# rbarile17/kelpie

Measured on AMD Instinct MI355X. Metric: candidate explanations evaluated/sec (incl. post-train) + rank-delta match rate, higher is better.
Workload: dtype bf16x3 (fp32-emulated)

## Files before the change

### include/kelpie_hip.h

```cpp
#ifndef KELPIE_HIP_H
#define KELPIE_HIP_H

#include <stddef.h>
#include <stdint.h>

#ifdef __cplusplus
extern "C" {
#endif

#define KP_OK 0
#define KP_EINVAL (-22)
#define KP_ENOMEM (-12)
#define KP_EDEVICE (-5)
#define KP_ENOTSUP (-95)
#define KP_INLINE 1

#define KP_MODEL_TRANSE 0
#define KP_MODEL_COMPLEX 1
#define KP_MODEL_CONVE 2

#define KP_OPT_ADAGRAD 0
#define KP_OPT_ADAM 1
#define KP_OPT_SGD 2

// ... 104 lines not shown
                        int32_t D, int32_t d, float xavier_std, int32_t n, const int32_t* R_base,
                        const int32_t* R_pt, const uint8_t* want, int32_t epochs, int32_t ratio,
                        int64_t n_entities, float* x_base, float* x_pt, int32_t* out);

int kp_rng_transe_calls_async(const uint8_t* torch_state, size_t torch_len, uint32_t* np_key, int32_t* np_pos,
                              int32_t normal_cap, int32_t D, int32_t d, float xavier_std, int32_t n,
                              const int32_t* R_base, const int32_t* R_pt, const uint8_t* want, int32_t epochs,
                              int32_t ratio, int64_t n_entities, float* x_base, float* x_pt, int32_t* out);

int kp_rng_torch_take(uint8_t* torch_state, size_t torch_len, int32_t* taken);

int kp_rng_wait(void);

int kp_rng_conve_masks(uint8_t* torch_state, size_t torch_len, int32_t n_steps, const int32_t* rows_per_step,
                       int32_t n_seg, const int32_t* seg_elems, const double* seg_keep, uint32_t* out_words);

int kp_rng_conve_masks_enqueue(uint8_t* torch_state, size_t torch_len, int32_t n_steps, const int32_t* rows_per_step,
                               int32_t n_seg, const int32_t* seg_elems, const double* seg_keep,
                               uint32_t* out_words);

int kp_last_timing(const kp_ctx* ctx, double* device_seconds, double* hot_kernel_seconds,
                   int64_t* hot_kernel_launches, double* hot_work_units);

int kp_hot_intervals(const kp_ctx* ctx, int64_t cap, double* out, int64_t* n);

typedef struct kp_graph kp_graph;
int kp_graph_create(int32_t n_ent, int64_t n_triples, const int32_t* triples, kp_graph** out);
void kp_graph_destroy(kp_graph* g);
const char* kp_graph_last_error(void);

int kp_graph_bfs(const kp_graph* g, int32_t n_src, const int32_t* src, int32_t* dist);

int kp_graph_set_classes(kp_graph* g, const int64_t* cls_off, const int32_t* cls);

int kp_graph_dijkstra_pairs(const kp_graph* g, int32_t n, const int32_t* src, const int32_t* dst, double* out);

typedef struct kp_view kp_view;
typedef struct kp_sched_batch kp_sched_batch;
int kp_view_create(int32_t kelpie, int32_t n_rel, int32_t original, const int32_t* base, int32_t n,
                   const int32_t* extra, int32_t m, kp_view** out);
void kp_view_destroy(kp_view* v);
int kp_sched_batch_create(kp_sched_batch** out);
void kp_sched_batch_destroy(kp_sched_batch* b);

int kp_sched_add_calls(kp_sched_batch* b, int32_t n, kp_view* const* views, const int32_t* rel, const uint8_t* flags,
                       const int32_t* cand_off, const int32_t* cands, int32_t* slot_idx, int32_t* n_rows,
// ... 14 lines not shown
```

### kelpie_amd/_lib.py

```python
from __future__ import annotations

import ctypes as C
import os
import sys
import weakref

import numpy as np

_HERE = os.path.dirname(os.path.abspath(__file__))
LIB_PATH = os.environ.get("KELPIE_HIP_LIB", os.path.join(_HERE, "libkelpie_hip.so"))

KP_MODEL = {"TransE": 0, "ComplEx": 1, "ConvE": 2}
KP_INLINE = 1
KP_OPT = {"Adagrad": 0, "Adam": 1, "SGD": 2}

EXPORTS = ["kp_ctx_create", "kp_ctx_destroy", "kp_last_error", "kp_posttrain_rank", "kp_all_scores",
           "kp_convertible", "kp_mt19937_discard", "kp_last_timing", "kp_version", "kp_rng_bernoulli_bits",
           "kp_rng_transe_epochs", "kp_rng_transe_enqueue", "kp_rng_wait", "kp_rng_batch_close", "kp_rng_batch_wait", "kp_rng_conve_masks", "kp_rng_conve_masks_enqueue", "kp_graph_create", "kp_graph_destroy",
           "kp_graph_last_error", "kp_graph_bfs", "kp_graph_set_classes", "kp_graph_dijkstra_pairs",
           "kp_predict_tails", "kp_dp_relevance", "kp_criage_relevance", "kp_hot_intervals", "kp_rng_normal",
           "kp_rng_transe_calls", "kp_train_epoch", "kp_read_tables", "kp_view_create", "kp_view_destroy",
           "kp_sched_batch_create", "kp_sched_batch_destroy", "kp_sched_add_calls", "kp_sched_pack",
           "kp_gather_i32", "kp_rng_transe_calls_async", "kp_rng_torch_take", "kp_conve_train_begin",
           "kp_conve_train_step", "kp_conve_train_read", "kp_host_alloc", "kp_host_free"]


class ModelDesc(C.Structure):
    _fields_ = [("model", C.c_int32), ("n_ent", C.c_int32), ("n_rel2", C.c_int32), ("dim", C.c_int32),
                ("entity", C.c_void_p), ("relation", C.c_void_p), ("conv_w", C.c_void_p), ("conv_b", C.c_void_p),
                ("fc_w", C.c_void_p), ("fc_b", C.c_void_p), ("bn_alpha", C.c_void_p), ("bn_beta", C.c_void_p),
                ("norm_p", C.c_int32)]


class HP(C.Structure):
    _fields_ = [("optimizer", C.c_int32), ("epochs", C.c_int32), ("batch_size", C.c_int32), ("lr", C.c_float),
                ("beta1", C.c_float), ("beta2", C.c_float), ("eps", C.c_float), ("reg_weight", C.c_float),
                ("margin", C.c_float), ("neg_ratio", C.c_int32), ("label_smoothing", C.c_float),
                ("hidden_dropout", C.c_float), ("input_dropout", C.c_float), ("fmap_dropout", C.c_float),
                ("reg_kind", C.c_int32)]


KP_REG = {"N3": 0, "N2": 1}


class Batch(C.Structure):
    _fields_ = [("n_slots", C.c_int32), ("x0", C.c_void_p), ("row_off", C.c_void_p), ("rows", C.c_void_p),
                ("rng_off", C.c_void_p), ("rng", C.c_void_p), ("pred", C.c_void_p), ("filt_off", C.c_void_p),
# ... 35 lines not shown
        L.kp_graph_destroy.restype = None
        L.kp_graph_last_error.restype = C.c_char_p
        L.kp_graph_bfs.argtypes = [C.c_void_p, C.c_int32, C.c_void_p, C.c_void_p]
        L.kp_graph_set_classes.argtypes = [C.c_void_p, C.c_void_p, C.c_void_p]
        L.kp_graph_dijkstra_pairs.argtypes = [C.c_void_p, C.c_int32, C.c_void_p, C.c_void_p, C.c_void_p]
        L.kp_rng_bernoulli_bits.argtypes = [C.c_void_p, C.c_size_t, C.c_uint64, C.c_double, C.c_void_p]
        L.kp_rng_transe_epochs.argtypes = [C.c_void_p, C.c_size_t, C.c_void_p, C.c_void_p, C.c_int32, C.c_int32,
                                           C.c_int32, C.c_int64, C.c_void_p]
        L.kp_rng_transe_enqueue.argtypes = L.kp_rng_transe_epochs.argtypes
        L.kp_rng_wait.argtypes = []
        L.kp_rng_batch_close.argtypes = [C.POINTER(C.c_int64)]
        L.kp_rng_batch_wait.argtypes = [C.c_int64]
        L.kp_train_epoch.argtypes = [C.c_void_p, C.POINTER(HP), C.c_int32, C.c_void_p, C.c_void_p, C.c_int32]
        L.kp_read_tables.argtypes = [C.c_void_p, C.c_void_p, C.c_void_p]
        L.kp_rng_normal.argtypes = [C.c_void_p, C.c_size_t, C.c_int64, C.c_float, C.c_float, C.c_int32, C.c_void_p]
        L.kp_rng_transe_calls.argtypes = [C.c_void_p, C.c_size_t, C.c_void_p, C.c_void_p, C.c_int32, C.c_int32,
                                          C.c_int32, C.c_float, C.c_int32, C.c_void_p, C.c_void_p, C.c_void_p,
                                          C.c_int32, C.c_int32, C.c_int64, C.c_void_p, C.c_void_p, C.c_void_p]
        L.kp_rng_conve_masks.argtypes = [C.c_void_p, C.c_size_t, C.c_int32, C.c_void_p, C.c_int32, C.c_void_p,
                                         C.c_void_p, C.c_void_p]
        L.kp_rng_conve_masks_enqueue.argtypes = L.kp_rng_conve_masks.argtypes
        L.kp_last_timing.argtypes = [C.c_void_p, C.POINTER(C.c_double), C.POINTER(C.c_double),
                                     C.POINTER(C.c_int64), C.POINTER(C.c_double)]
        L.kp_hot_intervals.argtypes = [C.c_void_p, C.c_int64, C.c_void_p, C.POINTER(C.c_int64)]
        L.kp_version.restype = C.c_char_p
        L.kp_view_create.argtypes = [C.c_int32, C.c_int32, C.c_int32, C.c_void_p, C.c_int32, C.c_void_p, C.c_int32,
                                     C.POINTER(C.c_void_p)]
        L.kp_view_destroy.argtypes = [C.c_void_p]
        L.kp_view_destroy.restype = None
        L.kp_sched_batch_create.argtypes = [C.POINTER(C.c_void_p)]
        L.kp_sched_batch_destroy.argtypes = [C.c_void_p]
        L.kp_sched_batch_destroy.restype = None
        L.kp_sched_add_calls.argtypes = [C.c_void_p, C.c_int32, C.c_void_p, C.c_void_p, C.c_void_p, C.c_void_p,
                                         C.c_void_p, C.c_void_p, C.c_void_p, C.c_void_p, C.c_void_p]
        L.kp_sched_pack.argtypes = [C.c_void_p, C.c_int32, C.c_void_p, C.c_void_p, C.c_int64, C.c_void_p,
                                    C.c_int64]
        L.kp_gather_i32.argtypes = [C.c_int32, C.c_void_p, C.c_void_p, C.c_void_p, C.c_int64]
        L.kp_rng_transe_calls_async.argtypes = L.kp_rng_transe_calls.argtypes
        L.kp_rng_torch_take.argtypes = [C.c_void_p, C.c_size_t, C.c_void_p]
        L.kp_conve_train_begin.argtypes = [C.c_void_p] * 5
        L.kp_conve_train_step.argtypes = [C.c_void_p, C.c_int32] + [C.c_void_p] * 6 + [C.c_float, C.c_float,
                                                                                      C.c_int32]
        L.kp_conve_train_read.argtypes = [C.c_void_p] * 9
        _LIB = L
    return _LIB

# ... 273 lines not shown
        check(lib().kp_dp_relevance(self.h, len(it), _ptr(it), float(epsilon), float(lambd), int(step_sign),
                                    int(rel_sign), _ptr(out)), self.h)
        return out

    def criage_relevance(self, items, ent_ids, tails_off, tails):
        it = np.ascontiguousarray(np.asarray(items, dtype=np.int32).reshape(-1, 5))
        ents = np.ascontiguousarray(ent_ids, dtype=np.int32)
        off = np.ascontiguousarray(tails_off, dtype=np.int32)
        tl = np.ascontiguousarray(np.asarray(tails, dtype=np.int32).reshape(-1, 2)) if len(tails) \
            else np.zeros((1, 2), np.int32)
        out = np.zeros(len(it), np.float64)
        status = np.zeros(len(it), np.int32)
        check(lib().kp_criage_relevance(self.h, len(it), _ptr(it), len(ents), _ptr(ents), _ptr(off), _ptr(tl),
                                        _ptr(out), _ptr(status)), self.h)
        return out, status

    def hot_intervals(self) -> np.ndarray:
        n = C.c_int64()
        check(lib().kp_hot_intervals(self.h, 0, None, C.byref(n)), self.h)
        out = np.zeros((max(1, n.value), 2), np.float64)
        check(lib().kp_hot_intervals(self.h, n.value, _ptr(out), C.byref(n)), self.h)
        return out[:n.value]

    def last_timing(self):
        a, b, n, w = C.c_double(), C.c_double(), C.c_int64(), C.c_double()
        check(lib().kp_last_timing(self.h, C.byref(a), C.byref(b), C.byref(n), C.byref(w)), self.h)
        return {"device_s": a.value, "hot_s": b.value, "hot_launches": n.value, "hot_work": w.value}


class Graph:

    def __init__(self, n_ent: int, triples):
        t = np.ascontiguousarray(np.asarray(triples, dtype=np.int32).reshape(-1, 3))
        h = C.c_void_p()
        self._lib = lib()
        self._check(self._lib.kp_graph_create(int(n_ent), len(t), _ptr(t), C.byref(h)))
        self._h = h
        self.n_ent = int(n_ent)

    def _check(self, rc):
        if rc != 0:
            raise KelpieHipError(f"libkelpie_hip error {rc}: {self._lib.kp_graph_last_error().decode()}")

    def __del__(self):
        h = getattr(self, "_h", None)
        if h is not None and h.value:
# ... 143 lines not shown
```

### kelpie_amd/csrc/kp_api.hip

```cpp
#include <cmath>
#include <cstdio>
#include <cstdlib>

#include "kp_common.hpp"

int cx_pick_db(int dim);

static thread_local std::string g_tls_err;

template <class F>
static int guarded(kp_ctx* c, F&& f) {
  try {
    f();
    if (c) c->err.clear();
    return KP_OK;
  } catch (const KpError& e) {
    if (c) c->err = e.msg;
    g_tls_err = e.msg;
    return e.code;
  } catch (const std::bad_alloc&) {
    if (c) c->err = "host out of memory";
    g_tls_err = "host out of memory";
    return KP_ENOMEM;
  } catch (...) {
// ... 77 lines not shown
    c->te_norm = m->norm_p == 1 ? 1 : 2;
    KP_HIP(hipSetDevice(device));
    KP_HIP(hipDeviceGetAttribute(&c->n_cu, hipDeviceAttributeMultiprocessorCount, device));
    (void)kp_time_base(device, nullptr);
    if (m->model == KP_MODEL_COMPLEX || m->model == KP_MODEL_CONVE) {
      KP_REQUIRE(m->model != KP_MODEL_COMPLEX || m->dim % 2 == 0, "ComplEx: row width must be even ([Re | Im])");
      int db = cx_pick_db(m->dim);
      KP_REQUIRE(db > 0, "row width > 400 not supported yet for ComplEx / ConvE");
      c->dp = 16 * db;
    } else {
      c->dp = round_up(m->dim, 16);
    }
    c->attn_mode = 1;
    if (const char* a = std::getenv("KP_ATTN")) c->attn_mode = std::strcmp(a, "f32") == 0 ? 0 : 1;
    c->cv_fused = 1;
    if (const char* a = std::getenv("KP_CV_FUSED")) c->cv_fused = std::atoi(a) != 0;
    c->cv_shared = 1;
    if (const char* a = std::getenv("KP_CV_SHARED")) c->cv_shared = std::atoi(a) != 0;
    if (const char* a = std::getenv("KP_CV_RANK")) c->cv_rank64 = std::strcmp(a, "f32") != 0;
    if (const char* a = std::getenv("KP_CV_DX")) c->cv_dx_block = std::strcmp(a, "block") == 0;
    if (const char* a = std::getenv("KP_TE_RANK")) c->te_rank64 = std::strcmp(a, "f32") != 0;
    if (const char* a = std::getenv("KP_ATTN_PART"))
      c->attn_part = std::strcmp(a, "streamk") == 0 ? 1 : std::strcmp(a, "ranges") == 0 ? 2 : 0;
    KP_HIP(hipStreamCreateWithFlags(&c->stream, hipStreamNonBlocking));
    {
      hipMemPool_t pool = device_pool(device);
      for (DevBuf* d : c->buffers()) {
        d->s = c->stream;
        d->pool = pool;
      }
    }
    KP_HIP(hipEventCreate(&c->ev0));
    KP_HIP(hipEventCreate(&c->ev1));
    upload_padded(c, &c->dE, m->entity, m->n_ent, m->dim, c->dp);
    upload_padded(c, &c->dR, m->relation, m->n_rel2, m->dim, c->dp);
    if (m->model == KP_MODEL_CONVE) {
      KP_REQUIRE(m->conv_w && m->conv_b && m->fc_w && m->fc_b && m->bn_alpha && m->bn_beta,
                 "ConvE: missing frozen layers");
      KP_REQUIRE(m->dim % 20 == 0 && m->dim / 20 >= 3, "ConvE: dim must be 20*h with h >= 3");
      c->hidden = 32 * 38 * (m->dim / 20 - 2);
      upload_plain(&c->d_conv_w, m->conv_w, 32 * 9);
      upload_plain(&c->d_conv_b, m->conv_b, 32);
      upload_plain(&c->d_fc_w, m->fc_w, (size_t)m->dim * c->hidden);
      upload_plain(&c->d_fc_b, m->fc_b, m->dim);
      upload_plain(&c->d_bn_a, m->bn_alpha, 1 + 32 + m->dim);
      upload_plain(&c->d_bn_b, m->bn_beta, 1 + 32 + m->dim);
// ... 211 lines not shown
                        const int32_t* tails_off, const int32_t* tails, double* out, int32_t* status) {
  if (!c || n < 0 || n_ents < 0 || (n > 0 && (!items || !out || !status || n_ents == 0)) ||
      (n_ents > 0 && (!ent_ids || !tails_off)))
    return KP_EINVAL;
  return guarded(c, [&] {
    if (n == 0) return;
    KP_HIP(hipSetDevice(c->device));
    criage_relevance(c, n, items, n_ents, ent_ids, tails_off, tails, out, status);
  });
}


int kp_hot_intervals(const kp_ctx* c, int64_t cap, double* out, int64_t* n) {
  if (!c || cap < 0 || (cap > 0 && !out)) return KP_EINVAL;
  const int64_t have = (int64_t)(c->hot_iv.size() / 2);
  if (n) *n = have;
  for (int64_t i = 0; i < std::min(cap, have); ++i) {
    out[2 * i] = c->hot_iv[2 * i];
    out[2 * i + 1] = c->hot_iv[2 * i + 1];
  }
  return KP_OK;
}

int kp_last_timing(const kp_ctx* c, double* dev_s, double* hot_s, int64_t* hot_n, double* hot_w) {
  if (!c) return KP_EINVAL;
  if (hot_w) *hot_w = c->timing.hot_work;
  if (dev_s) *dev_s = c->timing.device_s;
  if (hot_s) *hot_s = c->timing.hot_s;
  if (hot_n) *hot_n = c->timing.hot_launches;
  return KP_OK;
}

}
```

### kelpie_amd/csrc/kp_attn.hpp

```cpp
#pragma once
#if (defined(KP_ATTN_NODMA) || defined(KP_DIAG_M0SAVE)) && !defined(KP_DIAGNOSTIC_BUILD)
#error "KP_ATTN_NODMA is a timing-only diagnostic (wrong results): build it with make diag"
#endif
#include <algorithm>

#include "kp_common.hpp"

namespace kpattn {

#ifdef KP_ATTN_STAMPS
__device__ unsigned long long g_attn_stamps[8];
#define KP_STAMP(v) v = __builtin_amdgcn_s_memtime()
#else
#define KP_STAMP(v) (void)0
#endif

constexpr float kNegInf = -__builtin_huge_valf();

__device__ __forceinline__ float cx_q(const float* __restrict__ lhs, const float* __restrict__ rel, int d,
                                      int half) {
  if (d < half) {
    float ac = __fmul_rn(lhs[d], rel[d]);
    float be = __fmul_rn(lhs[d + half], rel[d + half]);
    return __fsub_rn(ac, be);
  } else if (d < 2 * half) {
    int i = d - half;
    float ae = __fmul_rn(lhs[i], rel[d]);
    float bc = __fmul_rn(lhs[d], rel[i]);
// ... 21 lines not shown
  return v;
}
__device__ __forceinline__ float lds_rd32(uint32_t addr) {
  float v;
  asm volatile("ds_read_b32 %0, %1" : "=v"(v) : "v"(addr));
  return v;
}
template <int N>
__device__ __forceinline__ void lgkm_wait() {
  asm volatile("s_waitcnt lgkmcnt(%0)" ::"n"(N));
}
__device__ __forceinline__ f32x4 tied(f32x4 v) {
  asm volatile("" : "+v"(v));
  return v;
}
__device__ __forceinline__ float tied(float v) {
  asm volatile("" : "+v"(v));
  return v;
}

enum { ATT_SOFTMAX_O = 0, ATT_SOFTMAX = 1, ATT_BCE_O = 2 };
constexpr float kMargin = 40.0f;

struct AttnWork {
  int ktq;
  int per_wg;
  int n_parts;
  int ranges;
};

template <int DB, int MODE>
__global__ __launch_bounds__(256, 1) void kp_attn(const float* __restrict__ E, int n_ent,
                                                  const float* __restrict__ Qpre, int nq, AttnWork wk,
                                                  float* __restrict__ out_m, float* __restrict__ out_l,
                                                  float* __restrict__ out_O, const float* __restrict__ qscale,
                                                  float ylo) {
  constexpr bool WITH_O = MODE != ATT_SOFTMAX;
  constexpr int DP = 16 * DB;
  constexpr int NSUB = 2;
  constexpr int KT = 16 * NSUB;
  constexpr int F4_ROW = DP / 4;
  constexpr int SEGS = (F4_ROW + 63) / 64;
  constexpr int S = 256 * SEGS + 4;
  extern __shared__ __attribute__((aligned(16))) float lds[];

  const int tid = threadIdx.x;
  const int lane = tid & 63;
  const int w = __builtin_amdgcn_readfirstlane(tid >> 6);
  const int g = lane >> 4, c = lane & 15;
  int key_begin = 0, key_end = 0;
  const uint32_t lds0 = (uint32_t)(uintptr_t)(__attribute__((address_space(3))) float*)lds;

// ... 207 lines not shown
              make_float4(O[4 * m][r], O[4 * m + 1][r], O[4 * m + 2][r], O[4 * m + 3][r]);
#pragma unroll
        for (int k = 0; k < DB % 4; ++k) dst[64 * (DB / 4) + 16 * k + i] = O[4 * (DB / 4) + k][r];
      }
    }
  }
  if (kt1 == wk.ktq && valid) {
    for (int pp = part + 1; pp < wk.n_parts; ++pp) {
      const size_t o = (size_t)pp * nq + q;
      if (g == 0 && MODE != ATT_BCE_O) {
        out_m[o] = kNegInf;
        out_l[o] = 0.f;
      }
      if (WITH_O) {
        float* dst = out_O + o * DP;
        for (int d = 4 * g; d < DP; d += 16) *reinterpret_cast<float4*>(dst + d) = make_float4(0.f, 0.f, 0.f, 0.f);
      }
    }
  }
  it += kt1 - kt0;
  }
}

struct AttnPlan {
  AttnWork wk;
  int n_wg;
};
inline AttnPlan attn_plan(int nq, int n_ent, int slots) {
  const int QT = (nq + 63) / 64, ktq = (n_ent + 31) / 32;
  const long long total = (long long)QT * ktq;
  long long per = (total + slots - 1) / slots;
  per = std::max<long long>(per, (ktq + 14) / 15);
  per = std::max<long long>(per, 1);
  AttnPlan p{};
  p.n_wg = (int)((total + per - 1) / per);
  p.wk.ktq = ktq;
  p.wk.per_wg = (int)per;
  int parts = 1;
  for (int qt = 0; qt < QT; ++qt) {
    const long long w0 = ((long long)qt * ktq) / per, w1 = ((long long)(qt + 1) * ktq - 1) / per;
    parts = std::max(parts, (int)(w1 - w0 + 1));
  }
  p.wk.n_parts = parts;
  return p;
}

inline AttnPlan attn_plan_ranges(int nq, int n_ent, int slots) {
  const int QT = (nq + 63) / 64, ktq = (n_ent + 31) / 32;
  const int n_wg = std::max(8, slots / 8 * 8);
  int best_s = 1;
  long long best = -1;
  for (int S = 1; S <= std::min(16, ktq); ++S) {
    const long long rounds = ((long long)QT * S + n_wg - 1) / n_wg;
    const long long cost = rounds * ((ktq + S - 1) / S + 2);
    if (best < 0 || cost < best) {
      best = cost;
      best_s = S;
    }
  }
  AttnPlan p{};
  p.wk.ktq = ktq;
  p.wk.per_wg = 0;
  p.wk.n_parts = best_s;
  p.wk.ranges = best_s;
  p.n_wg = (int)std::min<long long>(n_wg, ((long long)QT * best_s + 7) / 8 * 8);
  return p;
}

constexpr size_t attn_lds_bytes(int DB) {
  return 2u * 32u * (256u * ((4u * DB + 63u) / 64u) + 4u) * sizeof(float);
}

}
```

### kelpie_amd/csrc/kp_attn3.hpp

```cpp
#pragma once
#include <type_traits>

#include "kp_attn.hpp"

#ifdef KP_ATTN3_STAMPS
#ifndef KP_DIAGNOSTIC_BUILD
#error "KP_ATTN3_STAMPS is a diagnostic build (make diag / tools/attn_micro.sh)"
#endif
__device__ unsigned long long g_attn3_stamps[8];
#define KP3_STAMP(v) v = __builtin_amdgcn_s_memtime()
#define KP3_ACC(i, a, b) st_acc[i] += (b) - (a)
#else
#define KP3_STAMP(v) (void)0
#define KP3_ACC(i, a, b) (void)0
#endif

#ifdef KP_ATTN3_CLOCK
#ifndef KP_DIAGNOSTIC_BUILD
#error "KP_ATTN3_CLOCK is a diagnostic build (tools/attn_micro.sh)"
#endif
__device__ unsigned long long g_attn3_clock[4096][4];
#endif

#ifndef KP_O_AHEAD
// ... 885 lines not shown
    double* pre = reinterpret_cast<double*>(c->e3pre.ensure(sizeof(double) * (size_t)(ntiles + 1) * DP));
    hipLaunchKernelGGL((kp_tile_sums<DP>), dim3((unsigned)ntiles), dim3((DP + 63) / 64 * 64), 0, c->stream, c->dE,
                       c->n_ent, ts);
    KP_HIP(hipGetLastError());
    hipLaunchKernelGGL((kp_tile_prefix<DP>), dim3((DP + 63) / 64), dim3(64), 0, c->stream, ts, ntiles, pre);
    KP_HIP(hipGetLastError());
    c->e3pre_ready = true;
  }
  return c->e3pre.as<double>();
}

template <int DB, int MODE = ATT_SOFTMAX_O>
int attn3_wpc(kp_ctx* c) {
  static_assert(MODE == ATT_SOFTMAX_O || MODE == ATT_BCE_O, "attn3_wpc: the launched O mode");
  int& slot = c->attn3_wpc[MODE == ATT_BCE_O ? 1 : 0];
  if (slot <= 0) {
    int n = 0;
    KP_HIP(hipOccupancyMaxActiveBlocksPerMultiprocessor(&n, kp_attn3<DB, MODE>, 256, attn3_lds_bytes(DB)));
    slot = std::max(1, n);
  }
  return slot;
}

inline AttnPlan attn_plan_ctx(const kp_ctx* c, int nq, int n_ent, int slots) {
  const AttnPlan sk = attn_plan(nq, n_ent, slots);
  if (c->attn_mode != 1 || c->attn_part == 1) return sk;
  const AttnPlan r = attn_plan_ranges(nq, n_ent, slots);
  if (c->attn_part == 2) return r;
  const long long QT = (nq + 63) / 64, S = r.wk.ranges, ktq = r.wk.ktq;
  const long long n_wg = std::max(8, slots / 8 * 8);
  const long long cost_r = (QT * S + n_wg - 1) / n_wg * ((ktq + S - 1) / S + 2);
  const long long cost_sk = (long long)sk.wk.per_wg + 2;
  (void)n_ent;
  return 100 * cost_r <= 140 * cost_sk ? r : sk;
}

template <int DB, int MODE>
void launch_attn3(kp_ctx* c, int n_ent, const float* Q, int nq, const AttnPlan& plan, float* m, float* l, float* O,
                  const float* qscale, float ylo) {
  KP_REQUIRE(n_ent == c->n_ent, "attn3: key count differs from the table's (tile prefix sums)");
  KP_REQUIRE((long long)(n_ent + 31) / 32 * 32 * split3_row_bytes(16 * DB) + 1024 < (1LL << 31),
             "attn3: table too large for the 32-bit buffer descriptor of the split image");
  const uint8_t* E3 = split3_image<DB>(c);
  const double* pre = tile_prefix<DB>(c);
  hipLaunchKernelGGL((kp_attn3<DB, MODE>), dim3(plan.n_wg), dim3(256), attn3_lds_bytes(DB), c->stream, E3, n_ent, Q,
                     nq, plan.wk, m, l, O, qscale, ylo, pre);
  KP_HIP(hipGetLastError());
}

}
```

### kelpie_amd/csrc/kp_common.hpp

```cpp
#pragma once

#include <hip/hip_runtime.h>

#include <algorithm>
#include <array>
#include <cstdint>
#include <cstring>
#include <mutex>
#include <string>
#include <tuple>
#include <utility>
#include <vector>

#include "../../include/kelpie_hip.h"

typedef float f32x4 __attribute__((ext_vector_type(4)));

#define KP_WAVE 64

struct KpError {
  int code;
  std::string msg;
};

// ... 148 lines not shown
  hipEvent_t ev0 = nullptr, ev1 = nullptr;
  int model = 0;
  int n_ent = 0, n_rel2 = 0, dim = 0, dp = 0;
  int hidden = 0;
  float* dE = nullptr;
  float* dR = nullptr;
  float* d_conv_w = nullptr;
  float* d_conv_b = nullptr;
  float* d_fc_w = nullptr;
  float* d_fc_wt = nullptr;
  float* d_fc_b = nullptr;
  float* d_bn_a = nullptr;
  float* d_bn_b = nullptr;
  std::vector<float> hE;
  RankWs rank;
  ComplexWs cx;
  TranseWs te;
  ConveWs cv;
  std::string err;
  Timing timing;
  bool time_hot = true;
  int attn_mode = 0;
  int attn_part = 0;
  bool e3_ready = false;
  bool e3pre_ready = false;
  bool eT_ready = false;
  int cv_fused = 1;
  int cv_rank64 = 1;
  int cv_dx_block = 0;
  int te_norm = 2;
  int te_rank64 = 1;
  bool cvf_ready = false;
  int cv_shared = 1;
  bool cv_shared_ready = false;
  int attn3_wpc[2] = {0, 0};
  kp_train_state* train = nullptr;
  kp_cv_train* cvtrain = nullptr;
  std::vector<hipEvent_t> evpool;
  std::vector<std::pair<double, double>> hot_pairs;
  std::vector<double> hot_iv;
  std::vector<DevBuf*> buffers() {
    std::vector<DevBuf*> v;
    auto add = [&v](auto list) { v.insert(v.end(), list.begin(), list.end()); };
    add(ImageBufs::all());
    add(rank.all());
    add(cx.all());
// ... 109 lines not shown
```

### kelpie_amd/csrc/kp_complex.hip

```cpp
#include <algorithm>
#include <cstdio>
#include <cstdlib>
#include <cmath>
#include <unordered_map>

#include "kp_attn.hpp"
#include "kp_attn3.hpp"
#include "kp_posttrain.hpp"

namespace {
using namespace kpattn;

struct CxPlan {
  int b, q_begin, q_count, t_begin, t_count, cnt_l, cnt_r, pad;
};
struct CxQuery {
  int rel, c, ck, tg_begin, tg_count, pad0, pad1, pad2;
};
struct CxTail {
  int pair, c;
};


__global__ void kp_cx_qpair(const float* __restrict__ E, const float* __restrict__ R, int dp, int half,
// ... 577 lines not shown
  int32_t* dTg = upload(c, c->cx.targets, targets.data(), targets.size());
  int2* dPairs = upload(c, c->cx.pairs, pairs.data(), pairs.size());
  int4* dActs = upload(c, c->cx.acts, acts.data(), acts.size());
  int4* dStepQ = upload(c, c->cx.stepq, stepq.data(), std::max<size_t>(1, stepq.size()));
  int4* dStepT = upload(c, c->cx.stept, stept.data(), std::max<size_t>(1, stept.size()));
  float* dContrib = reinterpret_cast<float*>(c->cx.contrib.ensure(sizeof(float) * (size_t)std::max(1, max_items) * DP));
  const int npq = (int)pqs.size(), npairs = (int)pairs.size();
  float* dTsum = reinterpret_cast<float*>(c->cx.tsum.ensure(sizeof(float) * (size_t)std::max(npq, 1) * DP));
  float* dQpair = reinterpret_cast<float*>(c->cx.qpair.ensure(sizeof(float) * (size_t)std::max(npairs, 1) * DP));
  float* dLsef = reinterpret_cast<float*>(c->cx.lsef.ensure(sizeof(float) * (size_t)std::max(npairs, 1)));

  const Rank64Dev r64 = rank64_buffers(c, ns);
  int32_t* dPred = upload(c, c->rank.pred, bt->pred, (size_t)ns * 3);
  const RankDev rk = upload_rank_inputs(c, bt);

  const int half = c->dim / 2;
  KP_HIP(hipEventRecord(c->ev0, c->stream));
  if (npq > 0) {
    hipLaunchKernelGGL(kp_cx_tsum, dim3(npq), dim3(128), 0, c->stream, c->dE, DP, dPq, npq, dTg, dTsum);
    KP_HIP(hipGetLastError());
  }
  int slots_attn = 0;
  CX_DISPATCH(DBV, slots_attn = attn_slots_db<DB>(c));
  const AttnPlan plan_pairs = attn_plan_ctx(c, std::max(npairs, 1), c->n_ent, slots_attn);
  const int split_pairs = plan_pairs.wk.n_parts;
  size_t att_rows = (size_t)std::max(npairs, 1) * split_pairs;
  std::vector<AttnPlan> step_plan(T);
  for (int t = 0; t < T; ++t) {
    const int nq = q_off[t + 1] - q_off[t];
    step_plan[t] = attn_plan_ctx(c, std::max(nq, 1), c->n_ent, slots_attn);
    att_rows = std::max(att_rows, (size_t)nq * step_plan[t].wk.n_parts);
  }
  float* dAm = reinterpret_cast<float*>(c->cx.am.ensure(sizeof(float) * att_rows));
  float* dAl = reinterpret_cast<float*>(c->cx.al.ensure(sizeof(float) * att_rows));
  float* dAO = reinterpret_cast<float*>(c->cx.ao.ensure(sizeof(float) * att_rows * DP));
  float* dQs = reinterpret_cast<float*>(c->cx.qs.ensure(sizeof(float) * (size_t)std::max(max_nq, 1) * DP));
  if (npairs > 0) {
    hipLaunchKernelGGL(kp_cx_qpair, dim3(npairs), dim3(128), 0, c->stream, c->dE, c->dR, DP, half, dPairs, npairs,
                       dQpair);
    KP_HIP(hipGetLastError());
    CX_DISPATCH(DBV, launch_attn<DB>(c, false, dQpair, npairs, plan_pairs, dAm, dAl, nullptr));
    hipLaunchKernelGGL(kp_cx_lse_merge, dim3((npairs + 255) / 256), dim3(256), 0, c->stream, npairs, split_pairs, dAm,
                       dAl, dLsef);
    KP_HIP(hipGetLastError());
  }

  CxOpt opt{};
  opt.kind = hp->optimizer;
  opt.lr = hp->lr;
  opt.b1 = hp->beta1;
  opt.b2 = hp->beta2;
  opt.eps = hp->eps;
  opt.one_minus_b1 = (float)(1.0 - (double)hp->beta1);
// ... 99 lines not shown
```

### kelpie_amd/csrc/kp_conve.hip

```cpp
#include <cstdio>
#include <cmath>
#include <unordered_map>

#include "kp_attn.hpp"
#include "kp_attn3.hpp"
#include "kp_cv_fused.hpp"
#include "kp_posttrain.hpp"

int cx_pick_db(int dim);

namespace {
using namespace kpattn;

using kpcvf::CvBits;
struct CvInst {
  int slot, rel, b, pos;
  CvBits mb;
  int tail_begin, tail_count;
};
struct CvFInst {
  int slot, fp, b, pos;
  CvBits mb;
};
struct CvAct {
// ... 863 lines not shown
  int4* dFch = upload(c, c->cv.fchunks, fchunks.data(), std::max<size_t>(1, fchunks.size()));
  float* dFpart = reinterpret_cast<float*>(c->cv.fpart.ensure(sizeof(float) * (size_t)std::max(1, max_fch) * c->dim));
  CvBits* dEncBits = upload(c, c->cv.enc_bits, enc_bits.data(), std::max<size_t>(1, enc_bits.size()));
  float* dgs = reinterpret_cast<float*>(c->cv.gscale.ensure(sizeof(float) * (size_t)std::max<size_t>(1, kinst.size())));
  {
    std::vector<float> gsv(kinst.size());
    for (size_t i = 0; i < kinst.size(); ++i) gsv[i] = 1.0f / (float)((long long)kinst[i].b * (long long)(K + 1));
    if (!gsv.empty())
      KP_HIP(hipMemcpyAsync(dgs, gsv.data(), sizeof(float) * gsv.size(), hipMemcpyHostToDevice, c->stream));
  }
  int attn_slots = c->n_cu * (DBV <= 13 ? 2 : 1);
  if (c->attn_mode == 1) {
    switch (DBV) {
      case 4: attn_slots = c->n_cu * attn3_wpc<4, ATT_BCE_O>(c); break;
      case 8: attn_slots = c->n_cu * attn3_wpc<8, ATT_BCE_O>(c); break;
      case 13: attn_slots = c->n_cu * attn3_wpc<13, ATT_BCE_O>(c); break;
      case 16: attn_slots = c->n_cu * attn3_wpc<16, ATT_BCE_O>(c); break;
      case 25: attn_slots = c->n_cu * attn3_wpc<25, ATT_BCE_O>(c); break;
      default: throw KpError{KP_ENOTSUP, "ConvE: unsupported padded dimension"};
    }
  }
  std::vector<AttnPlan> step_plan(T);
  size_t o_rows = 1;
  for (int t = 0; t < T; ++t) {
    const int nk = kin_off[t + 1] - kin_off[t];
    step_plan[t] = attn_plan_ctx(c, std::max(nk, 1), K, attn_slots);
    o_rows = std::max(o_rows, (size_t)nk * step_plan[t].wk.n_parts);
  }
  float* dO = reinterpret_cast<float*>(c->cv.o.ensure(sizeof(float) * o_rows * DP));
  float* ddfc = reinterpret_cast<float*>(c->cv.dfc.ensure(sizeof(float) * (size_t)mk * c->dim));
  float* dgk = reinterpret_cast<float*>(c->cv.gk.ensure(sizeof(float) * (size_t)mk));
  float* ddflat = reinterpret_cast<float*>(c->cv.dflat.ensure(sizeof(float) * (size_t)(fused ? 1 : mk) * c->hidden));
  float* ddl = reinterpret_cast<float*>(c->cv.dl.ensure(sizeof(float) * (size_t)n_dl * mk * DP));
  float* dWt = conve_fc_wt(c);
  const float s_in = kc.has_in ? kc.scale_in : 1.0f, s_fm = kc.has_fm ? kc.scale_fm : 1.0f;

  CvOpt opt{};
  opt.lr = hp->lr;
  opt.b1 = hp->beta1;
  opt.b2 = hp->beta2;
  opt.eps = hp->eps;
  opt.one_minus_b1 = (float)(1.0 - (double)hp->beta1);
  opt.one_minus_b2 = (float)(1.0 - (double)hp->beta2);
  int64_t launches = 0;
  c->hot_pairs.clear();
  c->hot_iv.clear();
  const size_t shm_attn = attn_lds_bytes(DP / 16);
  const size_t shm_cbwd = sizeof(float) * 32 * 20 * (c->dim / 20 - 2);
  for (int t = 0; t < T; ++t) {
// ... 228 lines not shown
```

### kelpie_amd/engine.py

```python
from __future__ import annotations

import math
import os
import random
import time
from collections import OrderedDict
from dataclasses import dataclass, field

import numpy as np

from . import _lib
from .hparams import optimizer_hp
from .data import MANY_TO_ONE, ONE_TO_ONE, Dataset, KelpieView
from .models import FrozenModel
from .rng import ReferenceRNG, StateCheckpoint


def _sigmoid(x):
    return 1 / (1 + math.exp(-x))


@dataclass(slots=True)
class _Slot:
    x0: np.ndarray
# ... 485 lines not shown
        doff, nsz = a["doff"], a["nsz"]
        parts = [flat[doff[j]:doff[j] + nsz[j]] for j in js.tolist() if nsz[j]]
        return np.concatenate(parts).astype(np.int32, copy=False) if parts else np.zeros(1, np.int32)

    def _run_slots(self, slots, ctx, fill, gate=None):
        t_run = time.perf_counter()
        n = len(slots)
        ctx = ctx or self.model.ctx
        packed = self._pack(slots, ctx)
        if gate is not None and not gate():
            return None
        t_lib = time.perf_counter()
        score, rank, _ = ctx.posttrain_rank(self._kp_hp, *packed)
        t_end = time.perf_counter()
        if fill:
            for i, s in enumerate(slots):
                s.result = {"target_score": float(score[i]), "target_rank": int(rank[i])}
        stats = {"slots": n, "rows": int(packed[1][-1]), "pack_s": t_lib - t_run, "lib_s": t_end - t_lib,
                 **ctx.last_timing()}
        if not fill:
            stats["_score"], stats["_rank"] = np.array(score), np.array(rank)
        if hasattr(ctx, "hot_intervals"):
            stats["hot_iv"] = ctx.hot_intervals()
        self.last_batch_stats = stats
        return stats

    def _base_result(self, key, slots, pending_base):
        if key in self.base_pt_results:
            return self.base_pt_results[key]
        res = slots[pending_base[key]].result
        self.base_pt_results[key] = res
        return res

    def compute_relevance(self, pred, triples: list):
        return self.compute_relevance_batch(pred, [triples])[0]

    def compute_relevance_batch(self, pred, rules, checkpoints: list | None = None):
        raise NotImplementedError

    def _schedule_multi(self, items, checkpoints):
        raise NotImplementedError

    def _finalize_multi(self, slots, pending, jobs):
        raise NotImplementedError

    def _multi(self, items, checkpoints=None):
# ... 141 lines not shown
                    finally:
                        st["done"].set()

        class _Handle:
            def __init__(self, worker, st):
                self.ev = st["done"] = threading.Event()
                worker.q.put(st)

            def join(self):
                self.ev.wait()

            def is_alive(self):
                return not self.ev.is_set()

        workers = {}
        use_workers = os.environ.get("KELPIE_PIPELINE_WORKERS", "1") == "1"

        def run(state):
            try:
                b = state["b"]
                tr("run", b)
                _rng_mod.wait_ticket(state.get("ticket"))
                tr("draws", b)
                state["stats"] = dict(self._run(state["slots"], ctx=state["ctx"]))
                tr("ran", b)
            except BaseException as e:
                state["error"] = e

        tr("enter", -1)
        outs, stats, inflight = [], [], collections.deque()
        late_collect = os.environ.get("KELPIE_PIPELINE_EARLY_START", "1") == "0"
        detach = os.environ.get("KELPIE_PIPELINE_DETACH", "1") == "1"

        def finish(state):
            state["thread"].join()
            tr("finish", state["b"])
            if state.get("error") is not None:
                raise state["error"]
            self.base_pt_results = {}
            self._collect(state["slots"], state["stats"])
            o = self._finalize_multi(state["slots"], state["pending"], state["jobs"])
            st = state["stats"]
            st["schedule_s"] = state["schedule_s"]
            stats.append(st)
            outs.append(o)
            self._deferred_error = state.get("deferred")
            tr("finished", state["b"])
            self._raise_deferred(state["slots"], state["pending"])

        lookahead = max(0, int(os.environ.get("KELPIE_PIPELINE_LOOKAHEAD", "0")))
        ready = collections.deque()
        todo = iter(enumerate(batches))
        stop = False

        def schedule_next():
            nonlocal stop
            nxt = next(todo, None)
            if nxt is None:
                stop = True
                return False
            b, items = nxt
            self.set_cache()
            t0 = time.perf_counter()
            tr("schedule", b)
            self._deferred_error = None
            with self.rng.deferred(detach=detach) as drng:
                slots, pending, jobs = self._schedule_all(items, None)
            err, self._deferred_error = self._deferred_error, None
            tr("scheduled", b)
            ready.append({"slots": slots, "pending": pending, "jobs": jobs,
                          "schedule_s": time.perf_counter() - t0, "error": None, "deferred": err,
                          "ticket": drng.last_ticket, "b": b})
            if err is not None:
                stop = True
            return True

        def start_next(done):
            if late_collect or any(d.get("error") is not None for d in done):
                for d in done:
                    finish(d)
                done = []
            state = ready.popleft()
            state["ctx"] = ctxs[state["b"] % len(ctxs)]
            ci = state["b"] % len(ctxs)
            if not use_workers:
                state["thread"] = threading.Thread(target=run, args=(state,), daemon=True)
                state["thread"].start()
            else:
                if ci not in workers:
                    workers[ci] = _Worker()
                state["thread"] = _Handle(workers[ci], state)
            inflight.append(state)
            for d in done:
                finish(d)

        def join_oldest():
            old = inflight.popleft()
            old["thread"].join()
            tr("joined", old["b"])
            return old

        try:
            while True:
                if ready and (len(inflight) < len(ctxs) or not inflight[0]["thread"].is_alive()):
                    start_next([join_oldest()] if len(inflight) >= len(ctxs) else [])
                elif not stop and len(ready) <= lookahead:
# ... 174 lines not shown
```

Measured before the change: 923.4.

## Plan attention split for concurrent contexts when batches overlap in the pipeline

Adds an in-flight hint so that when several contexts run batches concurrently, the attention range split is sized to fill only a fraction of the device's workgroup slots (one-shot ranges plan) rather than assuming exclusive use of the GPU. The pipeline sets the hint to the number of contexts for middle batches and resets it afterwards. Planning code moves into a separate header, and plan diagnostics plus a KP_ATTN_RANGES override are exposed. ConvE keeps the old behaviour unless a compile flag is set. The risk is under-filling the GPU when overlap doesn't actually occur, or picking a worse split than the cost-model-based ranges plan.

After: 960.3 (median of 6 runs). 4.0% higher.

```diff
diff --git a/include/kelpie_hip.h b/include/kelpie_hip.h
--- a/include/kelpie_hip.h
+++ b/include/kelpie_hip.h
@@ -150,6 +150,10 @@
 int kp_last_timing(const kp_ctx* ctx, double* device_seconds, double* hot_kernel_seconds,
                    int64_t* hot_kernel_launches, double* hot_work_units);
 
+int kp_ctx_set_inflight(kp_ctx* ctx, int n);
+
+int kp_last_attn_plan(const kp_ctx* ctx, int32_t out[5]);
+
 int kp_hot_intervals(const kp_ctx* ctx, int64_t cap, double* out, int64_t* n);
 
 typedef struct kp_graph kp_graph;
diff --git a/kelpie_amd/_lib.py b/kelpie_amd/_lib.py
--- a/kelpie_amd/_lib.py
+++ b/kelpie_amd/_lib.py
@@ -22,7 +22,8 @@
            "kp_rng_transe_calls", "kp_train_epoch", "kp_read_tables", "kp_view_create", "kp_view_destroy",
            "kp_sched_batch_create", "kp_sched_batch_destroy", "kp_sched_add_calls", "kp_sched_pack",
            "kp_gather_i32", "kp_rng_transe_calls_async", "kp_rng_torch_take", "kp_conve_train_begin",
-           "kp_conve_train_step", "kp_conve_train_read", "kp_host_alloc", "kp_host_free"]
+           "kp_conve_train_step", "kp_conve_train_read", "kp_host_alloc", "kp_host_free", "kp_ctx_set_inflight",
+           "kp_last_attn_plan"]
 
 
 class ModelDesc(C.Structure):
@@ -104,6 +105,8 @@
         L.kp_rng_conve_masks_enqueue.argtypes = L.kp_rng_conve_masks.argtypes
         L.kp_last_timing.argtypes = [C.c_void_p, C.POINTER(C.c_double), C.POINTER(C.c_double),
                                      C.POINTER(C.c_int64), C.POINTER(C.c_double)]
+        L.kp_ctx_set_inflight.argtypes = [C.c_void_p, C.c_int]
+        L.kp_last_attn_plan.argtypes = [C.c_void_p, C.POINTER(C.c_int32)]
         L.kp_hot_intervals.argtypes = [C.c_void_p, C.c_int64, C.c_void_p, C.POINTER(C.c_int64)]
         L.kp_version.restype = C.c_char_p
         L.kp_view_create.argtypes = [C.c_int32, C.c_int32, C.c_int32, C.c_void_p, C.c_int32, C.c_void_p, C.c_int32,
@@ -423,6 +426,15 @@
         check(lib().kp_hot_intervals(self.h, n.value, _ptr(out), C.byref(n)), self.h)
         return out[:n.value]
 
+    def set_inflight(self, n: int):
+        check(lib().kp_ctx_set_inflight(self.h, int(n)), self.h)
+
+    def last_attn_plan(self):
+        v = (C.c_int32 * 5)()
+        check(lib().kp_last_attn_plan(self.h, v), self.h)
+        return {"attn_inflight": v[0], "attn_ranges": v[1], "attn_parts": v[2], "attn_wg": v[3],
+                "attn_queries": v[4]}
+
     def last_timing(self):
         a, b, n, w = C.c_double(), C.c_double(), C.c_int64(), C.c_double()
         check(lib().kp_last_timing(self.h, C.byref(a), C.byref(b), C.byref(n), C.byref(w)), self.h)
diff --git a/kelpie_amd/csrc/kp_api.hip b/kelpie_amd/csrc/kp_api.hip
--- a/kelpie_amd/csrc/kp_api.hip
+++ b/kelpie_amd/csrc/kp_api.hip
@@ -123,6 +123,7 @@
     if (const char* a = std::getenv("KP_TE_RANK")) c->te_rank64 = std::strcmp(a, "f32") != 0;
     if (const char* a = std::getenv("KP_ATTN_PART"))
       c->attn_part = std::strcmp(a, "streamk") == 0 ? 1 : std::strcmp(a, "ranges") == 0 ? 2 : 0;
+    if (const char* a = std::getenv("KP_ATTN_RANGES")) c->attn_ranges = std::max(0, std::min(16, std::atoi(a)));
     KP_HIP(hipStreamCreateWithFlags(&c->stream, hipStreamNonBlocking));
     {
       hipMemPool_t pool = device_pool(device);
@@ -380,6 +381,23 @@
   return KP_OK;
 }
 
+int kp_ctx_set_inflight(kp_ctx* c, int n) {
+  if (!c || n < 1) return KP_EINVAL;
+  c->attn_inflight = n;
+  return KP_OK;
+}
+
+int kp_last_attn_plan(const kp_ctx* c, int32_t out[5]) {
+  if (!c || !out) return KP_EINVAL;
+  const bool any = c->attn_last.nq >= 0;
+  out[0] = any ? c->attn_last.inflight : 0;
+  out[1] = any ? c->attn_last.ranges : 0;
+  out[2] = any ? c->attn_last.n_parts : 0;
+  out[3] = any ? c->attn_last.n_wg : 0;
+  out[4] = any ? c->attn_last.nq : 0;
+  return KP_OK;
+}
+
 int kp_last_timing(const kp_ctx* c, double* dev_s, double* hot_s, int64_t* hot_n, double* hot_w) {
   if (!c) return KP_EINVAL;
   if (hot_w) *hot_w = c->timing.hot_work;
diff --git a/kelpie_amd/csrc/kp_attn.hpp b/kelpie_amd/csrc/kp_attn.hpp
--- a/kelpie_amd/csrc/kp_attn.hpp
+++ b/kelpie_amd/csrc/kp_attn.hpp
@@ -4,6 +4,7 @@
 #endif
 #include <algorithm>
 
+#include "kp_attn_plan.hpp"
 #include "kp_common.hpp"
 
 namespace kpattn {
@@ -71,12 +72,6 @@
 enum { ATT_SOFTMAX_O = 0, ATT_SOFTMAX = 1, ATT_BCE_O = 2 };
 constexpr float kMargin = 40.0f;
 
-struct AttnWork {
-  int ktq;
-  int per_wg;
-  int n_parts;
-  int ranges;
-};
 
 template <int DB, int MODE>
 __global__ __launch_bounds__(256, 1) void kp_attn(const float* __restrict__ E, int n_ent,
@@ -330,51 +325,6 @@
   }
 }
 
-struct AttnPlan {
-  AttnWork wk;
-  int n_wg;
-};
-inline AttnPlan attn_plan(int nq, int n_ent, int slots) {
-  const int QT = (nq + 63) / 64, ktq = (n_ent + 31) / 32;
-  const long long total = (long long)QT * ktq;
-  long long per = (total + slots - 1) / slots;
-  per = std::max<long long>(per, (ktq + 14) / 15);
-  per = std::max<long long>(per, 1);
-  AttnPlan p{};
-  p.n_wg = (int)((total + per - 1) / per);
-  p.wk.ktq = ktq;
-  p.wk.per_wg = (int)per;
-  int parts = 1;
-  for (int qt = 0; qt < QT; ++qt) {
-    const long long w0 = ((long long)qt * ktq) / per, w1 = ((long long)(qt + 1) * ktq - 1) / per;
-    parts = std::max(parts, (int)(w1 - w0 + 1));
-  }
-  p.wk.n_parts = parts;
-  return p;
-}
-
-inline AttnPlan attn_plan_ranges(int nq, int n_ent, int slots) {
-  const int QT = (nq + 63) / 64, ktq = (n_ent + 31) / 32;
-  const int n_wg = std::max(8, slots / 8 * 8);
-  int best_s = 1;
-  long long best = -1;
-  for (int S = 1; S <= std::min(16, ktq); ++S) {
-    const long long rounds = ((long long)QT * S + n_wg - 1) / n_wg;
-    const long long cost = rounds * ((ktq + S - 1) / S + 2);
-    if (best < 0 || cost < best) {
-      best = cost;
-      best_s = S;
-    }
-  }
-  AttnPlan p{};
-  p.wk.ktq = ktq;
-  p.wk.per_wg = 0;
-  p.wk.n_parts = best_s;
-  p.wk.ranges = best_s;
-  p.n_wg = (int)std::min<long long>(n_wg, ((long long)QT * best_s + 7) / 8 * 8);
-  return p;
-}
-
 constexpr size_t attn_lds_bytes(int DB) {
   return 2u * 32u * (256u * ((4u * DB + 63u) / 64u) + 4u) * sizeof(float);
 }
diff --git a/kelpie_amd/csrc/kp_attn3.hpp b/kelpie_amd/csrc/kp_attn3.hpp
--- a/kelpie_amd/csrc/kp_attn3.hpp
+++ b/kelpie_amd/csrc/kp_attn3.hpp
@@ -931,17 +931,22 @@
   return slot;
 }
 
-inline AttnPlan attn_plan_ctx(const kp_ctx* c, int nq, int n_ent, int slots) {
-  const AttnPlan sk = attn_plan(nq, n_ent, slots);
-  if (c->attn_mode != 1 || c->attn_part == 1) return sk;
-  const AttnPlan r = attn_plan_ranges(nq, n_ent, slots);
-  if (c->attn_part == 2) return r;
-  const long long QT = (nq + 63) / 64, S = r.wk.ranges, ktq = r.wk.ktq;
-  const long long n_wg = std::max(8, slots / 8 * 8);
-  const long long cost_r = (QT * S + n_wg - 1) / n_wg * ((ktq + S - 1) / S + 2);
-  const long long cost_sk = (long long)sk.wk.per_wg + 2;
-  (void)n_ent;
-  return 100 * cost_r <= 140 * cost_sk ? r : sk;
+#ifndef KP_CV_ATTN_INFLIGHT
+#define KP_CV_ATTN_INFLIGHT 0
+#endif
+
+inline AttnPlan attn_plan_ctx(const kp_ctx* c, int nq, int n_ent, int slots, bool inflight_ok) {
+  if (c->attn_mode != 1) return attn_plan(nq, n_ent, slots);
+  return attn_plan_select(c->attn_part, inflight_ok ? c->attn_inflight : 1, c->attn_ranges, nq, n_ent, slots);
+}
+
+inline void attn_plan_note(kp_ctx* c, const AttnPlan& p, int nq, bool inflight_ok) {
+  if (nq < c->attn_last.nq) return;
+  c->attn_last.nq = nq;
+  c->attn_last.inflight = (c->attn_mode == 1 && inflight_ok) ? c->attn_inflight : 1;
+  c->attn_last.ranges = p.wk.ranges;
+  c->attn_last.n_parts = p.wk.n_parts;
+  c->attn_last.n_wg = p.n_wg;
 }
 
 template <int DB, int MODE>
diff --git a/kelpie_amd/csrc/kp_attn_plan.hpp b/kelpie_amd/csrc/kp_attn_plan.hpp
--- /dev/null
+++ b/kelpie_amd/csrc/kp_attn_plan.hpp
@@ -0,0 +1,110 @@
+#pragma once
+#include <algorithm>
+
+namespace kpattn {
+
+struct AttnWork {
+  int ktq;
+  int per_wg;
+  int n_parts;
+  int ranges;
+};
+
+struct AttnPlan {
+  AttnWork wk;
+  int n_wg;
+};
+inline AttnPlan attn_plan(int nq, int n_ent, int slots) {
+  const int QT = (nq + 63) / 64, ktq = (n_ent + 31) / 32;
+  const long long total = (long long)QT * ktq;
+  long long per = (total + slots - 1) / slots;
+  per = std::max<long long>(per, (ktq + 14) / 15);
+  per = std::max<long long>(per, 1);
+  AttnPlan p{};
+  p.n_wg = (int)((total + per - 1) / per);
+  p.wk.ktq = ktq;
+  p.wk.per_wg = (int)per;
+  int parts = 1;
+  for (int qt = 0; qt < QT; ++qt) {
+    const long long w0 = ((long long)qt * ktq) / per, w1 = ((long long)(qt + 1) * ktq - 1) / per;
+    parts = std::max(parts, (int)(w1 - w0 + 1));
+  }
+  p.wk.n_parts = parts;
+  return p;
+}
+
+constexpr int kAttnUnitOverhead = 2;
+#ifndef KP_ATTN_FILL_PCT
+#define KP_ATTN_FILL_PCT 75
+#endif
+constexpr int kAttnInflightFillPct = KP_ATTN_FILL_PCT;
+
+inline AttnPlan attn_plan_ranges(int nq, int n_ent, int slots) {
+  const int QT = (nq + 63) / 64, ktq = (n_ent + 31) / 32;
+  const int n_wg = std::max(8, slots / 8 * 8);
+  int best_s = 1;
+  long long best = -1;
+  for (int S = 1; S <= std::min(16, ktq); ++S) {
+    const long long rounds = ((long long)QT * S + n_wg - 1) / n_wg;
+    const long long cost = rounds * ((ktq + S - 1) / S + kAttnUnitOverhead);
+    if (best < 0 || cost < best) {
+      best = cost;
+      best_s = S;
+    }
+  }
+  AttnPlan p{};
+  p.wk.ktq = ktq;
+  p.wk.per_wg = 0;
+  p.wk.n_parts = best_s;
+  p.wk.ranges = best_s;
+  p.n_wg = (int)std::min<long long>(n_wg, ((long long)QT * best_s + 7) / 8 * 8);
+  return p;
+}
+
+inline AttnPlan attn_plan_oneshot(int nq, int n_ent, int S) {
+  const int QT = (nq + 63) / 64, ktq = (n_ent + 31) / 32;
+  S = std::max(1, std::min(S, std::min(16, ktq)));
+  AttnPlan p{};
+  p.wk.ktq = ktq;
+  p.wk.per_wg = 0;
+  p.wk.n_parts = S;
+  p.wk.ranges = S;
+  p.n_wg = (int)(((long long)QT * S + 7) / 8 * 8);
+  return p;
+}
+
+inline long long attn_ranges_wg_time(int nq, int n_ent, int S) {
+  const long long QT = (nq + 63) / 64, ktq = (n_ent + 31) / 32;
+  return QT * S * ((ktq + S - 1) / S + kAttnUnitOverhead);
+}
+
+constexpr int kAttnInflightMaxTiles = 256;
+
+inline AttnPlan attn_plan_inflight(int nq, int n_ent, int slots, bool* applied = nullptr) {
+  const int QT = (nq + 63) / 64, ktq = (n_ent + 31) / 32;
+  const int n_slots = std::max(8, slots / 8 * 8);
+  const long long want = (long long)kAttnInflightFillPct * n_slots;
+  int S = 1;
+  while (S < std::min(16, ktq) && 100LL * QT * S < want) ++S;
+  const bool ok = (long long)QT * S <= n_slots && (ktq + S - 1) / S <= kAttnInflightMaxTiles;
+  if (applied) *applied = ok;
+  return ok ? attn_plan_oneshot(nq, n_ent, S) : attn_plan_ranges(nq, n_ent, slots);
+}
+
+inline AttnPlan attn_plan_select(int part, int inflight, int force_s, int nq, int n_ent, int slots) {
+  const AttnPlan sk = attn_plan(nq, n_ent, slots);
+  if (part == 1) return sk;
+  if (force_s > 0) return attn_plan_oneshot(nq, n_ent, force_s);
+  const long long QT = (nq + 63) / 64;
+  bool shared = false;
+  const AttnPlan r = inflight >= 2 ? attn_plan_inflight(nq, n_ent, slots, &shared) : attn_plan_ranges(nq, n_ent, slots);
+  if (part == 2) return r;
+  const long long S = r.wk.ranges, ktq = r.wk.ktq;
+  const long long n_wg = std::max(8, slots / 8 * 8);
+  const long long cost_r = shared ? (attn_ranges_wg_time(nq, n_ent, (int)S) + n_wg - 1) / n_wg
+                                  : (QT * S + n_wg - 1) / n_wg * ((ktq + S - 1) / S + kAttnUnitOverhead);
+  const long long cost_sk = (long long)sk.wk.per_wg + kAttnUnitOverhead;
+  return 100 * cost_r <= 140 * cost_sk ? r : sk;
+}
+
+}
diff --git a/kelpie_amd/csrc/kp_common.hpp b/kelpie_amd/csrc/kp_common.hpp
--- a/kelpie_amd/csrc/kp_common.hpp
+++ b/kelpie_amd/csrc/kp_common.hpp
@@ -194,6 +194,11 @@
   bool time_hot = true;
   int attn_mode = 0;
   int attn_part = 0;
+  int attn_inflight = 1;
+  int attn_ranges = 0;
+  struct AttnLast {
+    int nq = -1, inflight = 1, ranges = 0, n_parts = 0, n_wg = 0;
+  } attn_last;
   bool e3_ready = false;
   bool e3pre_ready = false;
   bool eT_ready = false;
diff --git a/kelpie_amd/csrc/kp_complex.hip b/kelpie_amd/csrc/kp_complex.hip
--- a/kelpie_amd/csrc/kp_complex.hip
+++ b/kelpie_amd/csrc/kp_complex.hip
@@ -623,13 +623,15 @@
   }
   int slots_attn = 0;
   CX_DISPATCH(DBV, slots_attn = attn_slots_db<DB>(c));
-  const AttnPlan plan_pairs = attn_plan_ctx(c, std::max(npairs, 1), c->n_ent, slots_attn);
+  const AttnPlan plan_pairs = attn_plan_ctx(c, std::max(npairs, 1), c->n_ent, slots_attn, true);
   const int split_pairs = plan_pairs.wk.n_parts;
   size_t att_rows = (size_t)std::max(npairs, 1) * split_pairs;
   std::vector<AttnPlan> step_plan(T);
+  c->attn_last = {};
   for (int t = 0; t < T; ++t) {
     const int nq = q_off[t + 1] - q_off[t];
-    step_plan[t] = attn_plan_ctx(c, std::max(nq, 1), c->n_ent, slots_attn);
+    step_plan[t] = attn_plan_ctx(c, std::max(nq, 1), c->n_ent, slots_attn, true);
+    if (nq > 0) attn_plan_note(c, step_plan[t], nq, true);
     att_rows = std::max(att_rows, (size_t)nq * step_plan[t].wk.n_parts);
   }
   float* dAm = reinterpret_cast<float*>(c->cx.am.ensure(sizeof(float) * att_rows));
diff --git a/kelpie_amd/csrc/kp_conve.hip b/kelpie_amd/csrc/kp_conve.hip
--- a/kelpie_amd/csrc/kp_conve.hip
+++ b/kelpie_amd/csrc/kp_conve.hip
@@ -909,9 +909,11 @@
   }
   std::vector<AttnPlan> step_plan(T);
   size_t o_rows = 1;
+  c->attn_last = {};
   for (int t = 0; t < T; ++t) {
     const int nk = kin_off[t + 1] - kin_off[t];
-    step_plan[t] = attn_plan_ctx(c, std::max(nk, 1), K, attn_slots);
+    step_plan[t] = attn_plan_ctx(c, std::max(nk, 1), K, attn_slots, KP_CV_ATTN_INFLIGHT != 0);
+    if (nk > 0) attn_plan_note(c, step_plan[t], nk, KP_CV_ATTN_INFLIGHT != 0);
     o_rows = std::max(o_rows, (size_t)nk * step_plan[t].wk.n_parts);
   }
   float* dO = reinterpret_cast<float*>(c->cv.o.ensure(sizeof(float) * o_rows * DP));
diff --git a/kelpie_amd/engine.py b/kelpie_amd/engine.py
--- a/kelpie_amd/engine.py
+++ b/kelpie_amd/engine.py
@@ -531,6 +531,8 @@
             stats["_score"], stats["_rank"] = np.array(score), np.array(rank)
         if hasattr(ctx, "hot_intervals"):
             stats["hot_iv"] = ctx.hot_intervals()
+        if hasattr(ctx, "last_attn_plan"):
+            stats.update(ctx.last_attn_plan())
         self.last_batch_stats = stats
         return stats
 
@@ -718,7 +720,15 @@
                 tr("run", b)
                 _rng_mod.wait_ticket(state.get("ticket"))
                 tr("draws", b)
-                state["stats"] = dict(self._run(state["slots"], ctx=state["ctx"]))
+                hint = state.get("inflight", 1)
+                if hint > 1 and hasattr(state["ctx"], "set_inflight"):
+                    state["ctx"].set_inflight(hint)
+                    try:
+                        state["stats"] = dict(self._run(state["slots"], ctx=state["ctx"]))
+                    finally:
+                        state["ctx"].set_inflight(1)
+                else:
+                    state["stats"] = dict(self._run(state["slots"], ctx=state["ctx"]))
                 tr("ran", b)
             except BaseException as e:
                 state["error"] = e
@@ -747,6 +757,7 @@
         lookahead = max(0, int(os.environ.get("KELPIE_PIPELINE_LOOKAHEAD", "0")))
         ready = collections.deque()
         todo = iter(enumerate(batches))
+        n_batches = len(batches) if hasattr(batches, "__len__") else None
         stop = False
 
         def schedule_next():
@@ -778,6 +789,7 @@
                 done = []
             state = ready.popleft()
             state["ctx"] = ctxs[state["b"] % len(ctxs)]
+            state["inflight"] = len(ctxs) if n_batches is not None and 0 < state["b"] < n_batches - 1 else 1
             ci = state["b"] % len(ctxs)
             if not use_workers:
                 state["thread"] = threading.Thread(target=run, args=(state,), daemon=True)
```
